# world-modelz/world-modelz

Measured on AMD Instinct MI355X. Metric: denoise-step latent-frames/sec (forward, 32x16x16 latent clips), higher is better.
Workload: dtype bf16; 1 GPU; BASELINE.json configs[3] per GPU: VqVideoDiffusionModel.forward, B=8 clips/GPU of 32x16x16 latents, codebook 1024, dim 256, dim_head 128, heads 1, extents 3,3,3, depth 4, mlp 256; clips_per_gpu=8, codebook=1024, parallelism=clips sharded over 1 rank(s), no data-path collective

## Files before the change

include/wmz.h:

```cpp
#ifndef WMZ_H_
#define WMZ_H_

#include <stdint.h>

#ifdef __cplusplus
extern "C" {
#endif

#define WMZ_VERSION 115

enum { WMZ_F32 = 0, WMZ_BF16 = 1,
       WMZ_F16 = 2  };
enum { WMZ_OK = 0, WMZ_ERR_ARG = 1, WMZ_ERR_HIP = 2, WMZ_ERR_UNSUPPORTED = 3 };

enum {
  WMZ_LIN_GELU = 1,
  WMZ_LIN_GELU_IN = 2,
  WMZ_LIN_DGELU = 4
};

int wmz_version(void);
const char* wmz_last_error(void);

enum { WMZ_HG_STREAM = 1 , WMZ_HG_QKV = 2 ,
       WMZ_HG_CONV = 4  };
int wmz_half_guard_bind(void* word);
int wmz_half_guard_clear(void* word, void* stream);

int wmz_local3d_attn_fwd(const void* q, const void* k, const void* v, void* out, float* lse, float* logits_dbg,
                         int B, int S, int H, int W, int heads, int dh, int eS, int eH, int eW,
                         long ldq, long ldk, long ldv, long ldo, int dtype, void* stream);

int wmz_local3d_attn_fwd_general(const void* q, const void* k, const void* v, void* out, float* lse, float* logits_dbg,
                                 int B, int S, int H, int W, int heads, int dh, int eS, int eH, int eW,
                                 long ldq, long ldk, long ldv, long ldo, int dtype, void* stream);

int wmz_local3d_attn_bwd(const void* q, const void* k, const void* v, const void* out, const float* lse,
                         const void* dout, void* dq, void* dk, void* dv, float* delta_ws,
                         int B, int S, int H, int W, int heads, int dh, int eS, int eH, int eW,
                         long ldq, long ldk, long ldv, long ldo, long lddo, long lddq, long lddk, long lddv,
                         int dtype, void* stream);

int wmz_local3d_attn_bwd_general(const void* q, const void* k, const void* v, const void* out, const float* lse,
                                 const void* dout, void* dq, void* dk, void* dv, float* delta_ws,
                                 int B, int S, int H, int W, int heads, int dh, int eS, int eH, int eW,
                                 long ldq, long ldk, long ldv, long ldo, long lddo, long lddq, long lddk, long lddv,
                                 int dtype, void* stream);

int wmz_linear_fwd(const void* A, long lda, const void* Wt, const float* bias, const void* residual, long ldr,
                   void* C, long ldc, int M, int N, int K, const float* ln_gamma, const float* ln_beta,
                   float ln_eps, int flags, int out_f32, int dtype, void* stream);

int wmz_linear_fwd_stats(const void* A, long lda, const void* Wt, const float* bias, const void* residual, long ldr,
                         void* C, long ldc, int M, int N, int K, const float* ln_gamma, const float* ln_beta,
                         const float* ln_mean, const float* ln_rstd, float ln_eps, int flags, int out_f32, int dtype,
                         void* stream);

int wmz_linear_fwd_gelu_pair(const void* A, long lda, const void* Wt, const float* bias, void* Z, long ldz, void* H, long ldh,
                             int M, int N, int K, const float* ln_gamma, const float* ln_beta, const float* ln_mean,
                             const float* ln_rstd, float ln_eps, int dtype, void* stream);
int wmz_linear_fwd_train(const void* A, long lda, const void* Wt, const float* bias, void* C, long ldc, void* H, long ldh,
                         void* An, long ldan, int M, int N, int K, const float* ln_gamma, const float* ln_beta,
                         const float* ln_mean, const float* ln_rstd, float ln_eps, int dtype, void* stream);

int wmz_linear_fwd_blocked(const void* A, long lda, int rows_per_block, long block_stride, const void* Wt,
                           const float* bias, void* C, long ldc, int M, int N, int K, int out_f32, int dtype, void* stream);

long wmz_linear_wgrad_workspace_floats(int M, int N, int K, int dtype);
int wmz_linear_wgrad_ws(const void* dC, long ldc, const void* A, long lda, float* dW, float* dbias, int M, int N, int K,
                        const float* ln_gamma, const float* ln_beta, const float* ln_mean, const float* ln_rstd,
                        int gelu_in, int overwrite, float* workspace, long workspace_floats, int dtype, void* stream);
int wmz_linear_wgrad_batch(int n, const void* const* dC, const long* ldc, const void* const* A, const long* lda,
                           float* const* dW, float* const* dbias, const int* M, const int* N, const int* K,
                           const int* overwrite, const int* a_tiled, float* workspace, long workspace_floats, int dtype,
                           void* stream);
int wmz_linear_wgrad_batch_ln(int n, const void* const* dC, const long* ldc, const void* const* A, const long* lda,
                              float* const* dW, float* const* dbias, const int* M, const int* N, const int* K,
                              const int* overwrite, const float* const* ln_gamma, const float* const* ln_beta,
                              const float* const* ln_mean, const float* const* ln_rstd, float* workspace, long workspace_floats,
                              int dtype, void* stream);
int wmz_layernorm_stats(const void* x, long ldx, float* mean, float* rstd, int M, int K, float eps, int dtype,
                        void* stream);
int wmz_layernorm_bwd(const void* x, long ldx, const void* dyhat, long lddy, const void* skip, long ldskip,
                      const void* skip2, long ldskip2, const float* gamma, void* dx, long lddx, float* dgamma,
                      float* dbeta, int M, int K, float eps, int dtype, void* stream);

int wmz_embed_pos3d_fwd(const int64_t* z, const float* emb, const float* pos_s, const float* pos_h,
                        const float* pos_w, void* x, int B, int S, int H, int W, int D, int num_classes,
                        int dtype, void* stream);
int wmz_embed_pos3d_bwd(const int64_t* z, const void* dx, float* demb, float* dpos_s, float* dpos_h, float* dpos_w,
                        int B, int S, int H, int W, int D, int num_classes, int dtype, void* stream);
long wmz_embed_pos3d_bwd_workspace_ints(int B, int S, int H, int W, int num_classes);
int wmz_embed_pos3d_bwd_sorted(const int64_t* z, const void* dx, float* demb, float* dpos_s, float* dpos_h, float* dpos_w,
                               int B, int S, int H, int W, int D, int num_classes, int* workspace, long workspace_ints,
                               int dtype, void* stream);

int wmz_embed_indexed_fwd(const int64_t* tok, const int64_t* pos, const float* emb, const float* pos_s,
                          const float* pos_h, const float* pos_w, void* x, long ntok, int S, int H, int W, int D,
                          int num_classes, int dtype, void* stream);
int wmz_embed_indexed_bwd(const int64_t* tok, const int64_t* pos, const void* dx, float* demb, float* dpos_s,
                          float* dpos_h, float* dpos_w, long ntok, int S, int H, int W, int D, int num_classes, int dtype,
                          void* stream);

int wmz_vq_argmin(const float* x, long ldx, const float* codebook, int64_t* idx, float* dist_min,
                  int N, int C, int E, void* stream);

long wmz_vq_argmin_screened_workspace_bytes(int N, int C, int E);
int wmz_vq_argmin_screened(const float* x, long ldx, const float* codebook, int64_t* idx, float* dist_min, int N, int C, int E,
                           void* workspace, long workspace_bytes, void* stream);
int wmz_vq_gather(const int64_t* idx, const float* codebook, void* out, long ldo, int N, int C, int E,
                  int dtype, void* stream);
long wmz_loss_partials_workspace_floats(void);
int wmz_vq_tail_fwd(const float* x, const float* q, const float* counts, void* st, float* partial, float* loss,
                    float* perplexity, long N, int E, int Ep, int C, int out_dtype, void* stream);
int wmz_vq_tail_bwd(const void* d_st, const float* x, const float* q, const float* g_loss, void* d_x, long N, int E, int Ep,
                    int in_dtype, int st_dtype, void* stream);
int wmz_recon_loss_fwd(const void* y, const float* target, float* partial, float* loss, long B, long HW, int C, int Cp,
                       int kind, int dtype, void* stream);
int wmz_recon_loss_bwd(const void* y, const float* target, const float* g_loss, void* d_y, long B, long HW, int C, int Cp,
                       int kind, int dtype, void* stream);
int wmz_vq_ema_stats(const float* x, long ldx, const int64_t* idx, const float* codebook, float* counts,
                     float* dw, float* sqerr, int N, int C, int E, void* stream);
long wmz_vq_ema_stats_workspace_ints(int N, int C);
int wmz_vq_ema_stats_sorted(const float* x, long ldx, const int64_t* idx, const float* codebook, float* counts, float* dw,
                            float* sqerr, int N, int C, int E, int* workspace, long workspace_ints, void* stream);
int wmz_vq_ema_update(float* embedding, float* cluster_size, float* activation_count, const float* counts,
                      const float* dw, int C, int E, double decay, double eps, void* stream);

int wmz_layer_fused_fwd(const void* o, const void* x, void* x_out, void* q_out, void* kv_out, const void* wpack,
                        const float* vec, int ntok, int D, int I, int M, int has_head, int has_tail, float eps,
                        void* stream);

int wmz_embed_qkv_fused_fwd(const int64_t* z, const float* emb, const float* pos_s, const float* pos_h,
                            const float* pos_w, void* x_out, void* q_out, void* kv_out, const void* wpack,
                            const float* vec, int B, int S, int H, int W, int D, int I, int M, int num_classes, float eps,
                            void* stream);

#define WMZ_FUSED_X_IN_TILED 1
#define WMZ_FUSED_X_OUT_TILED 2
#define WMZ_FUSED_X1_NORMALISED 4
#define WMZ_FUSED_XRM_NORMALISED 8
int wmz_local3d_attn_fwd_planes(const void* q, const void* k, const void* v, void* out, float* lse, int B, int S, int H,
                                int W, int heads, int dh, int eS, int eH, int eW, long ldq, long ldk, long ldv, long ldo,
                                int q_plane0, int q_planes, int dtype, void* stream);
int wmz_layer_fused_fwd_planes(const void* o, const void* x, void* x_out, void* q_out, void* kv_out, const void* wpack,
                               const float* vec, int B, int planes_out, int planes_in, int HW, int D, int I, int M,
                               int has_head, int has_tail, int xflags, float eps, void* stream);
int wmz_layer_chain_supported(int D, int I, int M, int* mc);
int wmz_layer_chain_slab_pieces(void);
// ... 239 lines not shown
```

world_modelz_amd/csrc/linear_fwd.hip:

```cpp
#include "wmz_common.h"

namespace {

constexpr int BN = 128, ROWB = 128, CPR = 8, NT = 256;

struct LinParams {
  const void* A; long lda;
  const void* Wt;
  const float* bias;
  const void* res; long ldr;
  void* C; long ldc;
  void* C2; long ldc2;
  void* An; long ldan;
  int M, N, K;
  const float* gamma; const float* beta; float eps;
  const float* mean; const float* rstd;
  int flags, out_f32;
  int nbn;
  int rpb; long bstride;
  int dma;
};

typedef const __attribute__((address_space(1))) void* gptr_t;
typedef __attribute__((address_space(3))) void* lptr_t;

template <int N>
__device__ __forceinline__ void lgkm_wait_for3(s16x8& a, s16x8& b, s16x8& c) {
  asm volatile("s_waitcnt lgkmcnt(%3)" : "+v"(a), "+v"(b), "+v"(c) : "n"(N) : "memory");
}

template <typename T> __device__ __forceinline__ const T* a_row(const LinParams& P, int m) {
  const T* A = reinterpret_cast<const T*>(P.A);
  if (P.rpb == 0) return A + (long)m * P.lda;
  const int blk = m / P.rpb;
  return A + (long)blk * P.bstride + (long)(m - blk * P.rpb) * P.lda;
}

template <typename T, int PRO, int BM>
__global__ __launch_bounds__(NT, 2) void linear_kernel(LinParams P) {
  constexpr bool LN = PRO == 1;
  constexpr int NJ = BM == 128 ? 2 : 1;
  constexpr int AI = BM / 32;
  constexpr int EPC = 16 / (int)sizeof(T);
  constexpr int BK = CPR * EPC;
  constexpr int KSTEPS = BK / 16;
  constexpr bool DMA_FORM = PRO == 0 && BM == 64 && sizeof(T) == 2;
  constexpr int SLAB = (BM + BN) * ROWB;
  __shared__ __attribute__((aligned(1024))) char tiles[(DMA_FORM ? 3 : 1) * SLAB];
  char* As = tiles;
  char* Bs = tiles + BM * ROWB;
  __shared__ float mean_s[BM], rstd_s[BM];

  const int tid = threadIdx.x, lane = tid & 63, wave = tid >> 6;
  const int lid = xcd_remap(blockIdx.x, gridDim.x);
  const int bm = lid / P.nbn, bn = lid - bm * P.nbn;
  const int m0 = bm * BM, n0 = bn * BN;
  const T* A = reinterpret_cast<const T*>(P.A);
  const T* Wt = reinterpret_cast<const T*>(P.Wt);
  const int K = P.K;

  if constexpr (LN) {
   if (P.mean != nullptr) {
    for (int r = tid; r < BM; r += NT) {
      const int gm = m0 + r < P.M ? m0 + r : P.M - 1;
      mean_s[r] = P.mean[gm];
      rstd_s[r] = P.rstd[gm];
    }
   } else {
    const int sub = tid & 7;
    for (int r = tid >> 3; r < BM; r += NT / 8) {
      const int gm = m0 + r;
      float sum = 0.f;
      if (gm < P.M) {
        const T* row = a_row<T>(P, gm);
        for (int c = sub; c * EPC < K; c += 8) {
          float f[EPC];
          Elem<T>::unpack(*reinterpret_cast<const i32x4*>(row + c * EPC), f);
#pragma unroll
          for (int i = 0; i < EPC; ++i) sum += f[i];
        }
      }
      sum += __shfl_xor(sum, 1); sum += __shfl_xor(sum, 2); sum += __shfl_xor(sum, 4);
      const float mean = sum / (float)K;
// ... 238 lines not shown
        }
        __syncthreads();
#pragma unroll
        for (int it = 0; it < RR / 16; ++it) {
          const int idx = tid + it * NT;
          const int rl = idx >> 4, ch = idx & 15;
          const int row = m0 + round * RR + rl, col = n0 + ch * 8;
          if (row >= P.M || col >= P.N) continue;
          const f32x4 a = *reinterpret_cast<const f32x4*>(stage + rl * BN + ch * 8);
          const f32x4 b = *reinterpret_cast<const f32x4*>(stage + rl * BN + ch * 8 + 4);
          float f[8] = {a[0], a[1], a[2], a[3], b[0], b[1], b[2], b[3]};
          if (f32_staged) {
            float* dstf = reinterpret_cast<float*>(P.C) + (long)row * P.ldc + col;
            if (col + 8 <= P.N) {
              *reinterpret_cast<f32x4*>(dstf) = a;
              *reinterpret_cast<f32x4*>(dstf + 4) = b;
            } else {
              for (int e = 0; e < 8 && col + e < P.N; ++e) dstf[e] = f[e];
            }
            continue;
          }
          T* dst = reinterpret_cast<T*>(P.C) + (long)row * P.ldc + col;
          if (col + 8 <= P.N) {
            if (R) {
              float r8[8];
              Elem<T>::unpack(*reinterpret_cast<const i32x4*>(R + (long)row * P.ldr + col), r8);
#pragma unroll
              for (int e = 0; e < 8; ++e) {
                if (dgelu) f[e] *= wmz_dgelu(r8[e]);
                else f[e] += r8[e];
              }
            }
            *reinterpret_cast<i32x4*>(dst) = Elem<T>::pack(f);
            if (P.C2) {
#pragma unroll
              for (int e = 0; e < 8; ++e) f[e] = wmz_gelu(f[e]);
              *reinterpret_cast<i32x4*>(reinterpret_cast<T*>(P.C2) + (long)row * P.ldc2 + col) = Elem<T>::pack(f);
            }
          } else {
            for (int e = 0; e < 8 && col + e < P.N; ++e) {
              float v = f[e];
              if (R) {
                const float rv = Elem<T>::to_f32(R[(long)row * P.ldr + col + e]);
                if (dgelu) v *= wmz_dgelu(rv);
                else v += rv;
              }
              dst[e] = Elem<T>::from_f32(v);
              if (P.C2) reinterpret_cast<T*>(P.C2)[(long)row * P.ldc2 + col + e] = Elem<T>::from_f32(wmz_gelu(v));
            }
          }
        }
      }
      return;
    }
  }
#pragma unroll
  for (int i = 0; i < 2; ++i)
#pragma unroll
    for (int j = 0; j < NJ; ++j) {
      const int col = n0 + wc + 32 * j + l31;
      if (col >= P.N) continue;
      const float bv = P.bias ? P.bias[col] : 0.f;
#pragma unroll
      for (int reg = 0; reg < 16; ++reg) {
        const int row = m0 + wr + 32 * i + (reg & 3) + 8 * (reg >> 2) + 4 * hh;
        if (row >= P.M) continue;
        float v = acc[i][j][reg] + bv;
        if (gelu) v = wmz_gelu(v);
        if (R) {
          const float rv = Elem<T>::to_f32(R[(long)row * P.ldr + col]);
          if (dgelu) {
            v *= wmz_dgelu(rv);
          } else {
            v += rv;
          }
        }
        if (P.out_f32) reinterpret_cast<float*>(P.C)[(long)row * P.ldc + col] = v;
        else reinterpret_cast<T*>(P.C)[(long)row * P.ldc + col] = Elem<T>::from_f32(v);
        if (P.C2) reinterpret_cast<T*>(P.C2)[(long)row * P.ldc2 + col] = Elem<T>::from_f32(wmz_gelu(v));
      }
    }
}

}

extern "C" int WMZ_FN(wmz_linear_fwd)(const void* A, long lda, const void* Wt, const float* bias, const void* residual,
                              long ldr, void* C, long ldc, int M, int N, int K, const float* ln_gamma,
                              const float* ln_beta, float ln_eps, int flags, int out_f32, int dtype, void* stream) {
  return WMZ_FN(wmz_linear_fwd_stats)(A, lda, Wt, bias, residual, ldr, C, ldc, M, N, K, ln_gamma, ln_beta, nullptr, nullptr, ln_eps,
                              flags, out_f32, dtype, stream);
}

static int g_linear_dma = 1;
#ifndef WMZ_OP16_F16
extern "C" int wmz_debug_linear_knobs(int dma) { g_linear_dma = dma; return WMZ_OK; }
#endif

struct LinRoute { bool small; int bm; int dma; };
static LinRoute linear_route(const LinParams& P, bool op16, bool ln, bool gin, int dma_knob) {
  LinRoute r;
  r.small = (long)wmz_cdiv(P.M, 128) * wmz_cdiv(P.N, BN) < (P.out_f32 ? 192 : 320) && (op16 || (!ln && !gin));
  r.bm = r.small ? 64 : 128;
  const uintptr_t al = (uintptr_t)P.A | (uintptr_t)P.Wt | (uintptr_t)(P.lda * 2) | (uintptr_t)(P.bstride * 2);
  r.dma = (r.small && op16 && !ln && !gin && P.K % 64 == 0 && (al & 15) == 0 && dma_knob) ? 1 : 0;
  return r;
}

#ifndef WMZ_OP16_F16
extern "C" int wmz_debug_linear_route(const void* A, long lda, const void* Wt, long block_stride, int M, int N, int K, int prologue,
                                      int out_f32, int dtype) {
  WMZ_REQUIRE(M > 0 && N > 0 && K > 0 && prologue >= 0 && prologue <= 2, "wmz_debug_linear_route: bad shape or prologue");
  WMZ_REQUIRE(dtype == WMZ_F32 || dtype == WMZ_BF16 || dtype == WMZ_F16, "wmz_debug_linear_route: bad dtype %d", dtype);
  LinParams P = {};
  P.A = A; P.lda = lda; P.Wt = Wt; P.bstride = block_stride; P.M = M; P.N = N; P.K = K; P.out_f32 = out_f32;
  const LinRoute r = linear_route(P, dtype != WMZ_F32, prologue == 1, prologue == 2, dtype == WMZ_F16 ? 1 : g_linear_dma);
  return r.bm | (r.dma << 8);
}
#endif

static int linear_launch(LinParams P, const float* ln_gamma, int flags, int dtype, hipStream_t st) {
  const bool ln = ln_gamma != nullptr;
  const bool gin = (flags & WMZ_LIN_GELU_IN) != 0;
  WMZ_REQUIRE(!(ln && gin), "wmz_linear_fwd: LayerNorm and GELU prologues are exclusive");
  P.nbn = wmz_cdiv(P.N, BN);
  const LinRoute route = linear_route(P, dtype == kOp16Dtype, ln, gin, g_linear_dma);
  const bool small = route.small;
  const int bm = route.bm;
  P.dma = route.dma;
  dim3 grid((unsigned)(wmz_cdiv(P.M, bm) * P.nbn)), block(NT);
  if (dtype == kOp16Dtype) {
    if (small && ln) hipLaunchKernelGGL((linear_kernel<bf16_t, 1, 64>), grid, block, 0, st, P);
    else if (small && gin) hipLaunchKernelGGL((linear_kernel<bf16_t, 2, 64>), grid, block, 0, st, P);
    else if (small) hipLaunchKernelGGL((linear_kernel<bf16_t, 0, 64>), grid, block, 0, st, P);
    else if (ln) hipLaunchKernelGGL((linear_kernel<bf16_t, 1, 128>), grid, block, 0, st, P);
    else if (gin) hipLaunchKernelGGL((linear_kernel<bf16_t, 2, 128>), grid, block, 0, st, P);
    else hipLaunchKernelGGL((linear_kernel<bf16_t, 0, 128>), grid, block, 0, st, P);
  } else {
    if (small) hipLaunchKernelGGL((linear_kernel<float, 0, 64>), grid, block, 0, st, P);
    else if (ln) hipLaunchKernelGGL((linear_kernel<float, 1, 128>), grid, block, 0, st, P);
    else if (gin) hipLaunchKernelGGL((linear_kernel<float, 2, 128>), grid, block, 0, st, P);
    else hipLaunchKernelGGL((linear_kernel<float, 0, 128>), grid, block, 0, st, P);
  }
  WMZ_LAUNCH_CHECK("wmz_linear_fwd");
  return WMZ_OK;
}

extern "C" int WMZ_FN(wmz_linear_fwd_stats)(const void* A, long lda, const void* Wt, const float* bias, const void* residual,
                                    long ldr, void* C, long ldc, int M, int N, int K, const float* ln_gamma,
                                    const float* ln_beta, const float* ln_mean, const float* ln_rstd, float ln_eps,
                                    int flags, int out_f32, int dtype, void* stream) {
  WMZ_REQUIRE(A && Wt && C, "wmz_linear_fwd: null tensor");
  WMZ_REQUIRE((ln_mean == nullptr) == (ln_rstd == nullptr), "wmz_linear_fwd: ln_mean and ln_rstd go together");
  WMZ_REQUIRE(ln_mean == nullptr || ln_gamma != nullptr, "wmz_linear_fwd: statistics without a LayerNorm prologue");
  WMZ_REQUIRE(M > 0 && N > 0 && K > 0, "wmz_linear_fwd: bad shape M=%d N=%d K=%d", M, N, K);
  WMZ_REQUIRE(K % 8 == 0 && lda % 8 == 0, "wmz_linear_fwd: K and lda must be multiples of 8 (K=%d lda=%ld)", K, lda);
  WMZ_REQUIRE(dtype == WMZ_F32 || dtype == kOp16Dtype, "wmz_linear_fwd: bad dtype %d", dtype);
  WMZ_REQUIRE((ln_gamma == nullptr) == (ln_beta == nullptr), "wmz_linear_fwd: ln_gamma and ln_beta go together");
  LinParams P;
  P.A = A; P.lda = lda; P.Wt = Wt; P.bias = bias; P.res = residual; P.ldr = ldr; P.C = C; P.ldc = ldc;
  P.M = M; P.N = N; P.K = K; P.gamma = ln_gamma; P.beta = ln_beta; P.eps = ln_eps; P.flags = flags;
  P.mean = ln_mean; P.rstd = ln_rstd;
  P.out_f32 = out_f32;
  P.rpb = 0; P.bstride = 0;
  P.C2 = nullptr; P.ldc2 = 0;
  P.An = nullptr; P.ldan = 0;
  return linear_launch(P, ln_gamma, flags, dtype, (hipStream_t)stream);
}

#ifndef WMZ_OP16_F16
extern "C" int wmz_linear_fwd_gelu_pair(const void* A, long lda, const void* Wt, const float* bias, void* Z, long ldz, void* H,
                                        long ldh, int M, int N, int K, const float* ln_gamma, const float* ln_beta,
                                        const float* ln_mean, const float* ln_rstd, float ln_eps, int dtype, void* stream) {
  WMZ_REQUIRE(A && Wt && Z && H, "wmz_linear_fwd_gelu_pair: null tensor");
  WMZ_REQUIRE((ln_mean == nullptr) == (ln_rstd == nullptr), "wmz_linear_fwd_gelu_pair: ln_mean and ln_rstd go together");
  WMZ_REQUIRE(ln_mean == nullptr || ln_gamma != nullptr, "wmz_linear_fwd_gelu_pair: statistics without a LayerNorm prologue");
  WMZ_REQUIRE(M > 0 && N > 0 && K > 0, "wmz_linear_fwd_gelu_pair: bad shape M=%d N=%d K=%d", M, N, K);
  WMZ_REQUIRE(K % 8 == 0 && lda % 8 == 0, "wmz_linear_fwd_gelu_pair: K and lda must be multiples of 8 (K=%d lda=%ld)", K, lda);
  WMZ_REQUIRE(dtype == WMZ_F32 || dtype == kOp16Dtype, "wmz_linear_fwd_gelu_pair: bad dtype %d", dtype);
  WMZ_REQUIRE((ln_gamma == nullptr) == (ln_beta == nullptr), "wmz_linear_fwd_gelu_pair: ln_gamma and ln_beta go together");
  LinParams P;
  P.A = A; P.lda = lda; P.Wt = Wt; P.bias = bias; P.res = nullptr; P.ldr = 0; P.C = Z; P.ldc = ldz;
  P.M = M; P.N = N; P.K = K; P.gamma = ln_gamma; P.beta = ln_beta; P.eps = ln_eps; P.flags = 0;
  P.mean = ln_mean; P.rstd = ln_rstd;
  P.out_f32 = 0;
  P.rpb = 0; P.bstride = 0;
  P.C2 = H; P.ldc2 = ldh;
  P.An = nullptr; P.ldan = 0;
  return linear_launch(P, ln_gamma, 0, dtype, (hipStream_t)stream);
}

extern "C" int wmz_linear_fwd_train(const void* A, long lda, const void* Wt, const float* bias, void* C, long ldc, void* H, long ldh,
                                    void* An, long ldan, int M, int N, int K, const float* ln_gamma, const float* ln_beta,
                                    const float* ln_mean, const float* ln_rstd, float ln_eps, int dtype, void* stream) {
  WMZ_REQUIRE(A && Wt && C && ln_gamma && ln_beta, "wmz_linear_fwd_train: null tensor (a LayerNorm prologue is required)");
  WMZ_REQUIRE((ln_mean == nullptr) == (ln_rstd == nullptr), "wmz_linear_fwd_train: ln_mean and ln_rstd go together");
  WMZ_REQUIRE(M > 0 && N > 0 && K > 0, "wmz_linear_fwd_train: bad shape M=%d N=%d K=%d", M, N, K);
  WMZ_REQUIRE(K % 8 == 0 && lda % 8 == 0 && (An == nullptr || ldan % 8 == 0), "wmz_linear_fwd_train: K, lda, ldan must be multiples of 8");
  WMZ_REQUIRE(dtype == WMZ_F32 || dtype == kOp16Dtype, "wmz_linear_fwd_train: bad dtype %d", dtype);
  LinParams P;
  P.A = A; P.lda = lda; P.Wt = Wt; P.bias = bias; P.res = nullptr; P.ldr = 0; P.C = C; P.ldc = ldc;
  P.M = M; P.N = N; P.K = K; P.gamma = ln_gamma; P.beta = ln_beta; P.eps = ln_eps; P.flags = 0;
  P.mean = ln_mean; P.rstd = ln_rstd;
  P.out_f32 = 0;
  P.rpb = 0; P.bstride = 0;
  P.C2 = H; P.ldc2 = ldh;
  P.An = An; P.ldan = ldan;
  return linear_launch(P, ln_gamma, 0, dtype, (hipStream_t)stream);
}

#endif

extern "C" int WMZ_FN(wmz_linear_fwd_blocked)(const void* A, long lda, int rows_per_block, long block_stride, const void* Wt,
                                      const float* bias, void* C, long ldc, int M, int N, int K, int out_f32, int dtype,
                                      void* stream) {
  WMZ_REQUIRE(A && Wt && C, "wmz_linear_fwd_blocked: null tensor");
  WMZ_REQUIRE(M > 0 && N > 0 && K > 0 && rows_per_block > 0, "wmz_linear_fwd_blocked: bad shape M=%d N=%d K=%d rows_per_block=%d", M, N, K, rows_per_block);
  WMZ_REQUIRE(K % 8 == 0 && lda % 8 == 0 && block_stride % 8 == 0, "wmz_linear_fwd_blocked: K, lda, block_stride must be multiples of 8");
  WMZ_REQUIRE(dtype == WMZ_F32 || dtype == kOp16Dtype, "wmz_linear_fwd_blocked: bad dtype %d", dtype);
  LinParams P;
  P.A = A; P.lda = lda; P.Wt = Wt; P.bias = bias; P.res = nullptr; P.ldr = 0; P.C = C; P.ldc = ldc;
  P.M = M; P.N = N; P.K = K; P.gamma = nullptr; P.beta = nullptr; P.eps = 0.f; P.flags = 0;
  P.mean = nullptr; P.rstd = nullptr;
  P.out_f32 = out_f32;
  P.rpb = rows_per_block; P.bstride = block_stride;
  P.C2 = nullptr; P.ldc2 = 0;
  P.An = nullptr; P.ldan = 0;
  return linear_launch(P, nullptr, 0, dtype, (hipStream_t)stream);
}
```

world_modelz_amd/csrc/wmz_debug.h:

```cpp
#pragma once
#ifdef __cplusplus
extern "C" {
#endif

int wmz_debug_fused_timestamps(void* buf);
int wmz_debug_fused_knobs(int dbg);
int wmz_debug_attn_timestamps(void* buf);
int wmz_debug_attn_knobs(int dbg, int variant);

int wmz_debug_conv_knobs(int skew, int dbg);

int wmz_debug_linear_knobs(int dma);
int wmz_debug_linear_route(const void* A, long lda, const void* Wt, long block_stride, int M, int N, int K, int prologue,
                           int out_f32, int dtype);

int wmz_debug_stamp(void* buf, int slot, void* stream);

int wmz_debug_conv_stamps(unsigned long long* out, int n);
int wmz_debug_w3_stamps(unsigned long long* out, int n);
int wmz_debug_attn_infer_stamps(unsigned long long* out, int n);

#ifdef __cplusplus
}
#endif
```

world_modelz_amd/functional.py:

```python
import torch

from . import _cast, ops
from .config import get_compute_dtype

LN_EPS = 1e-5


class _AttentionBlock(torch.autograd.Function):
    @staticmethod
    def forward(ctx, x_kv, x_q, ln_g, ln_b, wq, wk, wv, bv, wout, bout, residual, extents, heads, grad_on, same_src,
                res_is_xkv, out_f32=False):
        dt = x_kv.dtype
        I = wq.shape[0]
        ln = None if ln_g is None else (ln_g.detach(), ln_b.detach())
        wq_c = _cast.operand(wq, dt)
        wkv_c = _cast.operand((wk, wv), dt, 'kv', lambda a, b: torch.cat([a, b], dim=0))
        bkv = _cast.operand((bv,), torch.float32, 'bkv', lambda b: torch.cat([torch.zeros_like(b), b]))
        lead = x_q.shape[:-1]
        need_bwd = grad_on and any(ctx.needs_input_grad)
        stats = ops.layernorm_stats(x_kv, LN_EPS) if (need_bwd and ln is not None) else None
        q = ops.linear_fwd(x_q, wq_c)
        xn = None
        if stats is not None and x_kv.numel() // x_kv.shape[-1] >= ops.KEEP_NORM_MIN_ROWS:
            kv, _, xn = ops.linear_fwd_train(x_kv, wkv_c, bkv, ln, LN_EPS, stats, want_norm=True)
        else:
            kv = ops.linear_fwd(x_kv, wkv_c, bias=bkv, ln=ln, ln_eps=LN_EPS, ln_stats=stats)
        o, lse, _ = ops.local3d_attention_fwd(q, kv[..., :I], kv[..., I:], extents, heads, need_lse=need_bwd)
        if wout is not None:
            y = ops.linear_fwd(o, _cast.operand(wout, dt), bias=bout.detach(), residual=residual, out_f32=bool(out_f32) and not need_bwd)
        else:
            y = o if residual is None else o + residual
        if need_bwd:
            ctx.save_for_backward(x_kv, x_q, ln_g, ln_b, wq, wk, wv, bv, wout, bout, q, kv, o, lse)
            ctx.extents, ctx.heads, ctx.has_res = extents, heads, residual is not None
            ctx.ln_stats = stats
            ctx.xn = xn
            ctx.same_src, ctx.res_is_xkv = bool(same_src), bool(res_is_xkv)
        return y.reshape(*lead, y.shape[-1])

    @staticmethod
    def backward(ctx, dy):
        from . import backward as B
        return B.attention_block_backward(ctx, dy) + (None,)


class _FeedForwardBlock(torch.autograd.Function):
    @staticmethod
    def forward(ctx, x, ln_g, ln_b, w1, b1, w2, b2, residual, grad_on, res_is_x):
        dt = x.dtype
        ln = None if ln_g is None else (ln_g.detach(), ln_b.detach())
        need_bwd = grad_on and any(ctx.needs_input_grad)
        w1_c, w2_c = _cast.operand(w1, dt), _cast.operand(w2, dt)
        if need_bwd:
            stats = ops.layernorm_stats(x, LN_EPS) if ln is not None else None
            xn = None
            if ln is not None and x.numel() // x.shape[-1] >= ops.KEEP_NORM_MIN_ROWS:
                z, h, xn = ops.linear_fwd_train(x, w1_c, b1.detach(), ln, LN_EPS, stats, want_gelu=True, want_norm=True)
            else:
                z, h = ops.linear_fwd_gelu_pair(x, w1_c, bias=b1.detach(), ln=ln, ln_eps=LN_EPS, ln_stats=stats)
            y = ops.linear_fwd(h, w2_c, bias=b2.detach(), residual=residual)
            ctx.save_for_backward(x, ln_g, ln_b, w1, b1, w2, b2, z, h, xn)
            ctx.ln_stats = stats
            ctx.has_res = residual is not None
            ctx.res_is_x = bool(res_is_x)
        else:
            h = ops.linear_fwd(x, w1_c, bias=b1.detach(), ln=ln, ln_eps=LN_EPS, gelu=True)
            y = ops.linear_fwd(h, w2_c, bias=b2.detach(), residual=residual)
        return y

    @staticmethod
    def backward(ctx, dy):
        from . import backward as B
        return B.feed_forward_block_backward(ctx, dy)


class _Embed(torch.autograd.Function):
    @staticmethod
    def forward(ctx, z, emb, pos_s, pos_h, pos_w, dtype):
        x = ops.embed_pos3d_fwd(z, emb.detach(), pos_s.detach(), pos_h.detach(), pos_w.detach(), dtype)
        ctx.save_for_backward(z)
        ctx.params = (emb, pos_s, pos_h, pos_w)
        return x

    @staticmethod
    def backward(ctx, dx):
        from . import backward as B
        return B.embed_backward(ctx, dx)


class _Linear(torch.autograd.Function):

    @staticmethod
    def forward(ctx, x, w, b, out_f32):
        bias = None if b is None else b.detach()
        if x.dim() >= 3 and not x.is_contiguous() and x[0].is_contiguous() and x.stride(0) % 8 == 0:
            xb = x.view(x.shape[0], -1, x.shape[-1])
            y = ops.linear_fwd_blocks(xb, _cast.operand(w, x.dtype), bias, out_f32).view(*x.shape[:-1], w.shape[0])
        else:
            y = ops.linear_fwd(x, _cast.operand(w, x.dtype), bias=bias, out_f32=out_f32)
        ctx.save_for_backward(x, w, b)
        return y

    @staticmethod
    def backward(ctx, dy):
        from . import backward as B
        return B.linear_backward(ctx, dy)


def _as_compute(x):
    dt = get_compute_dtype()
    if not x.is_cuda:
        raise ops.L.WmzError('world_modelz_amd modules run on the GPU only (no CPU fallback); got a CPU tensor')
    return x if x.dtype == dt else x.to(dt)


def attention_block(x_kv, x_q, ln, wq, wk, wv, bv, wout, bout, residual, extents, heads, out_f32=False):
    g, b = (None, None) if ln is None else ln
    return _AttentionBlock.apply(x_kv, x_q, g, b, wq, wk, wv, bv, wout, bout, residual, tuple(int(e) for e in extents),
                                 int(heads), torch.is_grad_enabled(), x_q is x_kv, residual is x_kv, bool(out_f32))


def feed_forward_block(x, ln, w1, b1, w2, b2, residual):
    g, b = (None, None) if ln is None else ln
    return _FeedForwardBlock.apply(x, g, b, w1, b1, w2, b2, residual, torch.is_grad_enabled(), residual is x)


def embed_tokens(z, emb, pos_s, pos_h, pos_w):
    return _Embed.apply(z, emb, pos_s, pos_h, pos_w, get_compute_dtype())


def linear(x, w, b=None, out_f32=False):
    return _Linear.apply(x, w, b, out_f32)



def _dense_grid(n):
    if n % 16 == 0:
        return (1, n // 16, 16), (0, n // 16, 16)
    return (1, 1, n), (0, 0, n)


class _DenseAttentionBlock(torch.autograd.Function):

    @staticmethod
    def forward(ctx, x, ln_g, ln_b, wqkv, wout, bout, residual, heads, grad_on, res_is_x):
        dt = x.dtype
        B, n, _ = x.shape
        I = wqkv.shape[0] // 3
        ln = None if ln_g is None else (ln_g.detach(), ln_b.detach())
        need_bwd = grad_on and any(ctx.needs_input_grad)
        stats = ops.layernorm_stats(x, LN_EPS) if (ln is not None and need_bwd) else None
        qkv = ops.linear_fwd(x, _cast.operand(wqkv, dt), ln=ln, ln_eps=LN_EPS, ln_stats=stats)
        (S, H, W), ext = _dense_grid(n)
        g = qkv.view(B, S, H, W, 3 * I)
        o, lse, _ = ops.local3d_attention_fwd(g[..., :I], g[..., I:2 * I], g[..., 2 * I:], ext, heads, need_lse=need_bwd)
        o = o.view(B, n, I)
        if wout is not None:
            y = ops.linear_fwd(o, _cast.operand(wout, dt), bias=bout.detach(), residual=residual)
        else:
            y = o if residual is None else o + residual
        if need_bwd:
            ctx.save_for_backward(x, ln_g, ln_b, wqkv, wout, bout, qkv, o, lse)
            ctx.ln_stats = stats
            ctx.heads, ctx.has_res = heads, residual is not None
            ctx.res_is_x = bool(res_is_x)
        return y

    @staticmethod
    def backward(ctx, dy):
        from . import backward as Bk
        return Bk.dense_attention_block_backward(ctx, dy)


class _EmbedIndexed(torch.autograd.Function):
    @staticmethod
    def forward(ctx, tok, pos, emb, pos_s, pos_h, pos_w, shape, dtype):
        x = ops.embed_indexed_fwd(tok, pos, emb.detach(), pos_s.detach(), pos_h.detach(), pos_w.detach(), shape, dtype)
        ctx.save_for_backward(tok, pos)
# ... 28 lines not shown
```

world_modelz_amd/ops.py:

```python
import contextlib
import ctypes
import os

import torch

from . import _lib as L


def _rows(t):
    if t.stride(-1) != 1:
        t = t.contiguous()
    C = t.shape[-1]
    flat = t.reshape(-1, C) if t.is_contiguous() else None
    if flat is None:
        if t.dim() >= 2 and all(t.stride(i) == t.stride(i + 1) * t.shape[i + 1] for i in range(t.dim() - 2)):
            return t, t.numel() // C, t.stride(-2)
        t = t.contiguous()
        flat = t.reshape(-1, C)
    return t, flat.shape[0], C


def _out_rows(out, M, dtype):
    t, Mo, ld = _rows(out)
    assert Mo == M and t.data_ptr() == out.data_ptr() and out.dtype == dtype
# ... 46 lines not shown
    if ln_stats is not None:
        mean, rstd = ln_stats
        assert ln is not None and mean.numel() == M and rstd.numel() == M
    L.call(L.half_form('wmz_linear_fwd_stats', a.dtype), L.ptr(a), lda, L.ptr(weight), L.ptr(bias), L.ptr(residual), ldr, L.ptr(out), ldc,
           M, N, K, L.ptr(g), L.ptr(b), L.ptr(mean), L.ptr(rstd), float(ln_eps),
           (L.WMZ_LIN_GELU if gelu else 0) | (L.WMZ_LIN_GELU_IN if gelu_in else 0), 1 if out_f32 else 0, dt,
           L.stream())
    return out


KEEP_NORM_MIN_ROWS = 16384


def linear_fwd_train(a, weight, bias, ln, ln_eps=1e-5, ln_stats=None, want_gelu=False, want_norm=False, out=None):
    K = a.shape[-1]
    N = weight.shape[0]
    dt = L.dtype_code(a.dtype)
    assert weight.dtype == a.dtype and weight.is_contiguous() and weight.shape[1] == K and ln is not None
    a, M, lda = _rows(a)
    lead = a.shape[:-1]
    ldc = ldh = N
    ldan = K
    if out is not None:
        c, h, an = out
        assert (h is not None) == want_gelu and (an is not None) == want_norm
        c, ldc = _out_rows(c, M, a.dtype)
        if h is not None:
            h, ldh = _out_rows(h, M, a.dtype)
        if an is not None:
            an, ldan = _out_rows(an, M, a.dtype)
    else:
        c = torch.empty(lead + (N,), dtype=a.dtype, device=a.device)
        h = torch.empty(lead + (N,), dtype=a.dtype, device=a.device) if want_gelu else None
        an = torch.empty(lead + (K,), dtype=a.dtype, device=a.device) if want_norm else None
    g, b = ln
    mean = rstd = None
    if ln_stats is not None:
        mean, rstd = ln_stats
        assert mean.numel() == M and rstd.numel() == M
    assert bias is None or bias.dtype == torch.float32
    L.call('wmz_linear_fwd_train', L.ptr(a), lda, L.ptr(weight), L.ptr(bias), L.ptr(c), ldc, L.ptr(h), ldh, L.ptr(an), ldan, M, N, K,
           L.ptr(g), L.ptr(b), L.ptr(mean), L.ptr(rstd), float(ln_eps), dt, L.stream())
    return c, h, an


def linear_fwd_gelu_pair(a, weight, bias=None, ln=None, ln_eps=1e-5, ln_stats=None, out=None):
    K = a.shape[-1]
    N = weight.shape[0]
    dt = L.dtype_code(a.dtype)
    assert weight.dtype == a.dtype and weight.is_contiguous() and weight.shape[1] == K
    a, M, lda = _rows(a)
    lead = a.shape[:-1]
    ldz = ldh = N
    if out is not None:
        z, ldz = _out_rows(out[0], M, a.dtype)
        h, ldh = _out_rows(out[1], M, a.dtype)
    else:
        z = torch.empty(lead + (N,), dtype=a.dtype, device=a.device)
        h = torch.empty(lead + (N,), dtype=a.dtype, device=a.device)
    g = b = mean = rstd = None
    if ln is not None:
        g, b = ln
        assert g.dtype == torch.float32 and b.dtype == torch.float32
    if ln_stats is not None:
        mean, rstd = ln_stats
        assert ln is not None and mean.numel() == M and rstd.numel() == M
    assert bias is None or bias.dtype == torch.float32
    L.call('wmz_linear_fwd_gelu_pair', L.ptr(a), lda, L.ptr(weight), L.ptr(bias), L.ptr(z), ldz, L.ptr(h), ldh, M, N, K,
           L.ptr(g), L.ptr(b), L.ptr(mean), L.ptr(rstd), float(ln_eps), dt, L.stream())
    return z, h


def linear_fwd_blocks(a, weight, bias=None, out_f32=False, out=None):
    Bk, R, K = a.shape
    N = weight.shape[0]
    assert a.stride(2) == 1 and weight.dtype == a.dtype and weight.is_contiguous() and weight.shape[1] == K
    ldc = N
    if out is None:
        out = torch.empty((Bk, R, N), dtype=torch.float32 if out_f32 else a.dtype, device=a.device)
    else:
        out, ldc = _out_rows(out, Bk * R, torch.float32 if out_f32 else a.dtype)
    L.call(L.half_form('wmz_linear_fwd_blocked', a.dtype), L.ptr(a), a.stride(1), R, a.stride(0), L.ptr(weight), L.ptr(bias), L.ptr(out), ldc,
           Bk * R, N, K, 1 if out_f32 else 0, L.dtype_code(a.dtype), L.stream())
    return out


def embed_pos3d_fwd(z, emb, pos_s, pos_h, pos_w, dtype):
    B, S, H, W = z.shape
    D = emb.shape[1]
    z = z.contiguous()
    x = torch.empty((B, S, H, W, D), dtype=dtype, device=z.device)
    L.call('wmz_embed_pos3d_fwd', L.ptr(z), L.ptr(emb), L.ptr(pos_s), L.ptr(pos_h), L.ptr(pos_w), L.ptr(x),
           B, S, H, W, D, emb.shape[0], L.dtype_code(dtype), L.stream())
    return x


_vq_screen_ws = {}


def vq_argmin(x, codebook, need_dist=False, exact_scan=False):
    assert x.dtype == torch.float32 and codebook.dtype == torch.float32
    x, N, ldx = _rows(x)
    codebook = codebook.contiguous()
    C, E = codebook.shape
    idx = torch.empty((N,), dtype=torch.int64, device=x.device)
    dmin = torch.empty((N,), dtype=torch.float32, device=x.device) if need_dist else None
    need = 0 if (exact_scan or N == 0 or ldx % 4 or x.data_ptr() % 16) else L.lib().wmz_vq_argmin_screened_workspace_bytes(N, C, E)
    if need > 0:
        ws = _vq_screen_ws.get(x.device)
        if ws is None or ws.numel() < need:
            ws = _vq_screen_ws[x.device] = torch.empty(need, dtype=torch.uint8, device=x.device)
        L.call('wmz_vq_argmin_screened', L.ptr(x), ldx, L.ptr(codebook), L.ptr(idx), L.ptr(dmin), N, C, E, L.ptr(ws), ws.numel(),
               L.stream())
    else:
        L.call('wmz_vq_argmin', L.ptr(x), ldx, L.ptr(codebook), L.ptr(idx), L.ptr(dmin), N, C, E, L.stream())
    return (idx, dmin) if need_dist else idx


def vq_gather(idx, codebook, dtype=torch.float32):
    codebook = codebook.contiguous()
    C, E = codebook.shape
    flat = idx.reshape(-1).contiguous()
    out = torch.empty((flat.shape[0], E), dtype=dtype, device=idx.device)
    L.call('wmz_vq_gather', L.ptr(flat), L.ptr(codebook), L.ptr(out), E, flat.shape[0], C, E, L.dtype_code(dtype),
           L.stream())
    return out.reshape(*idx.shape, E)


_loss_partials = {}


def _partials(device):
    w = _loss_partials.get(device)
    if w is None:
        w = _loss_partials[device] = torch.empty(int(L.lib().wmz_loss_partials_workspace_floats()), dtype=torch.float32, device=device)
    return w


class _VqTail(torch.autograd.Function):

    @staticmethod
    def forward(ctx, inp, flat, q, counts, out_dtype, Ep):
        N, E = flat.shape
        dev = flat.device
        st = torch.empty(inp.shape[:-1] + (Ep,), dtype=out_dtype, device=dev)
        loss = torch.empty((), dtype=torch.float32, device=dev)
        ppl = torch.empty((), dtype=torch.float32, device=dev)
        L.call('wmz_vq_tail_fwd', L.ptr(flat), L.ptr(q), L.ptr(counts), L.ptr(st), L.ptr(_partials(dev)), L.ptr(loss), L.ptr(ppl),
               N, E, Ep, counts.numel(), L.dtype_code(out_dtype), L.stream())
        ctx.save_for_backward(flat, q)
        ctx.meta = (inp.shape, inp.dtype, Ep, out_dtype)
        ctx.mark_non_differentiable(ppl)
        return st, loss, ppl

    @staticmethod
    def backward(ctx, d_st, d_loss, _d_ppl):
        flat, q = ctx.saved_tensors
        shape, in_dtype, Ep, out_dtype = ctx.meta
        N, E = flat.shape
        if d_st is not None:
            d_st = d_st.contiguous()
            assert d_st.dtype == out_dtype
        if d_loss is not None:
            d_loss = d_loss.reshape(1).float()
        dx = torch.empty(shape, dtype=in_dtype, device=flat.device)
        L.call('wmz_vq_tail_bwd', L.ptr(d_st), L.ptr(flat), L.ptr(q), L.ptr(d_loss), L.ptr(dx), N, E, Ep, L.dtype_code(in_dtype),
# ... 913 lines not shown
```

Baseline: 821,800 latent-frames/s.

## Add specialized single-pass logits GEMM kernel for K=256 bf16 fp32-output projection

Adds a dedicated kernel for the final codebook logits projection (K=256, bf16 inputs, fp32 output). It loads the whole K extent for a 64x128 tile into LDS in one pass using direct global-to-LDS loads, runs MFMA over four K slabs with fine-grained waits, then stages the results through LDS so fp32 stores are coalesced. The Python linear path sends eligible out_f32 calls to it and falls back to the generic blocked linear otherwise. This targets the generic kernel's tiling overhead and uncoalesced fp32 output writes on a large M x 1024 output, at the cost of a single-occupancy, large-LDS kernel.

```diff
diff --git a/include/wmz.h b/include/wmz.h
--- a/include/wmz.h
+++ b/include/wmz.h
@@ -65,6 +65,11 @@
 
 int wmz_linear_fwd_blocked(const void* A, long lda, int rows_per_block, long block_stride, const void* Wt,
                            const float* bias, void* C, long ldc, int M, int N, int K, int out_f32, int dtype, void* stream);
+
+int wmz_logits_fwd(const void* A, long lda, int rows_per_block, long block_stride, const void* Wt, const float* bias, float* C,
+                   long ldc, int M, int N, int K, int dtype, void* stream);
+int wmz_logits_unit_takes(const void* A, long lda, int rows_per_block, long block_stride, const void* Wt, const void* C, long ldc,
+                          int M, int N, int K, int dtype);
 
 long wmz_linear_wgrad_workspace_floats(int M, int N, int K, int dtype);
 int wmz_linear_wgrad_ws(const void* dC, long ldc, const void* A, long lda, float* dW, float* dbias, int M, int N, int K,
diff --git a/world_modelz_amd/csrc/linear_fwd.hip b/world_modelz_amd/csrc/linear_fwd.hip
--- a/world_modelz_amd/csrc/linear_fwd.hip
+++ b/world_modelz_amd/csrc/linear_fwd.hip
@@ -1,4 +1,5 @@
 #include "wmz_common.h"
+#include "mem_policy.h"
 
 namespace {
 
@@ -403,6 +404,113 @@
     }
 }
 
+#ifndef WMZ_OP16_F16
+struct LogitsParams {
+  const char* A; long lda_b;
+  int rpb; long bstride_b;
+  const char* Wt;
+  const float* bias;
+  float* C; long ldc;
+  int nbn;
+};
+constexpr int LU_BM = 64, LU_K = 256, LU_SLABS = LU_K / 64;
+constexpr int LU_SLAB = (LU_BM + BN) * ROWB;
+constexpr int LU_PITCH = 40;
+constexpr int LU_STAGE = LU_BM * LU_PITCH * 4;
+constexpr int LU_LDS = LU_SLABS * LU_SLAB + 4 * LU_STAGE;
+
+__global__ __launch_bounds__(NT, 1) void logits_unit_kernel(LogitsParams P) {
+  extern __shared__ __attribute__((aligned(1024))) char lu_lds[];
+  const int tid = threadIdx.x, lane = tid & 63;
+  const int wave = __builtin_amdgcn_readfirstlane(tid >> 6);
+  const int lid = xcd_remap(blockIdx.x, gridDim.x);
+  const int bm = lid / P.nbn, bn = lid - bm * P.nbn;
+  const int m0 = bm * LU_BM, n0 = bn * BN;
+  const int blk = m0 / P.rpb;
+  const char* a0 = P.A + (long)blk * P.bstride_b + (long)(m0 - blk * P.rpb) * P.lda_b;
+  const char* w0 = P.Wt + (long)n0 * (LU_K * 2);
+  const int l31 = lane & 31, hh = lane >> 5;
+  const float bv = P.bias ? P.bias[n0 + wave * 32 + l31] : 0.f;
+
+  {
+    const int lr = lane >> 3, lc = lane & 7;
+    const char* asrc[2];
+    const char* bsrc[4];
+#pragma unroll
+    for (int q = 0; q < 2; ++q) {
+      const int r = 8 * (wave + 4 * q) + lr;
+      asrc[q] = a0 + (long)r * P.lda_b + ((lc ^ (swz128(r) >> 4)) << 4);
+    }
+#pragma unroll
+    for (int q = 0; q < 4; ++q) {
+      const int r = 8 * (wave + 4 * q) + lr;
+      bsrc[q] = w0 + r * (LU_K * 2) + ((lc ^ (swz128(r) >> 4)) << 4);
+    }
+#pragma unroll
+    for (int s = 0; s < LU_SLABS; ++s) {
+      char* dst = lu_lds + s * LU_SLAB;
+#pragma unroll
+      for (int q = 0; q < 2; ++q)
+        __builtin_amdgcn_global_load_lds((gptr_t)(asrc[q] + s * ROWB), (lptr_t)(dst + (wave + 4 * q) * 1024), 16, 0, 0);
+#pragma unroll
+      for (int q = 0; q < 4; ++q)
+        __builtin_amdgcn_global_load_lds((gptr_t)(bsrc[q] + s * ROWB), (lptr_t)(dst + LU_BM * ROWB + (wave + 4 * q) * 1024), 16, 0, 0);
+    }
+  }
+
+  f32x16 acc[2] = {(f32x16)(0.f), (f32x16)(0.f)};
+  unsigned aA[4];
+  {
+    const unsigned base = lds_addr(lu_lds) + (unsigned)l31 * ROWB;
+    const int t = (hh * 16) ^ swz128(l31);
+#pragma unroll
+    for (int kk = 0; kk < 4; ++kk) aA[kk] = base + (unsigned)((kk * 32) ^ t);
+  }
+  const unsigned wrow = (unsigned)(LU_BM * ROWB + wave * 32 * ROWB);
+  static_for<LU_SLABS>([&](auto sc) {
+    constexpr int S = decltype(sc)::value;
+    constexpr int OFF = (S & 1) * LU_SLAB;
+    asm volatile("s_waitcnt vmcnt(%0)" ::"n"(6 * (LU_SLABS - 1 - S)) : "memory");
+    __builtin_amdgcn_s_barrier();
+    s16x8 fa[4], fb[4], fw[4];
+    static_for<4>([&](auto kc) {
+      constexpr int kk = decltype(kc)::value;
+      const unsigned a = aA[kk] + (unsigned)((S >> 1) * 2 * LU_SLAB);
+      fa[kk] = ds_read_b128_asm<OFF>(a);
+      fb[kk] = ds_read_b128_asm<OFF + 32 * ROWB>(a);
+      fw[kk] = ds_read_b128_asm<OFF>(a + wrow);
+    });
+    static_for<4>([&](auto kc) {
+      constexpr int kk = decltype(kc)::value;
+      lgkm_wait_for3<3 * (3 - kk)>(fa[kk], fb[kk], fw[kk]);
+      Frag8<bf16_t> x0, x1, w;
+      x0.v = fa[kk]; x1.v = fb[kk]; w.v = fw[kk];
+      mma32(acc[0], x0, w);
+      mma32(acc[1], x1, w);
+    });
+  });
+
+  float* stage = reinterpret_cast<float*>(lu_lds + LU_SLABS * LU_SLAB + wave * LU_STAGE);
+#pragma unroll
+  for (int i = 0; i < 2; ++i)
+#pragma unroll
+    for (int reg = 0; reg < 16; ++reg)
+      stage[(32 * i + (reg & 3) + 8 * (reg >> 2) + 4 * hh) * LU_PITCH + l31] = acc[i][reg] + bv;
+  __builtin_amdgcn_fence(__ATOMIC_RELEASE, "wavefront");
+  __builtin_amdgcn_wave_barrier();
+  __builtin_amdgcn_fence(__ATOMIC_ACQUIRE, "wavefront");
+  char* cbase = reinterpret_cast<char*>(P.C + (long)m0 * P.ldc + n0 + wave * 32);
+  const int sr = lane >> 3, sch = lane & 7;
+  const unsigned ldc_b = (unsigned)P.ldc * 4u;
+#pragma unroll
+  for (int it = 0; it < LU_BM / 8; ++it) {
+    const int row = 8 * it + sr;
+    const f32x4 v = *reinterpret_cast<const f32x4*>(stage + row * LU_PITCH + 4 * sch);
+    gstore_at<MemPolicy::Plain>(cbase, (unsigned)row * ldc_b + (unsigned)sch * 16u, 0, v);
+  }
+}
+#endif
+
 }
 
 extern "C" int WMZ_FN(wmz_linear_fwd)(const void* A, long lda, const void* Wt, const float* bias, const void* residual,
@@ -548,3 +656,37 @@
   P.An = nullptr; P.ldan = 0;
   return linear_launch(P, nullptr, 0, dtype, (hipStream_t)stream);
 }
+
+#ifndef WMZ_OP16_F16
+extern "C" int wmz_logits_unit_takes(const void* A, long lda, int rows_per_block, long block_stride, const void* Wt, const void* C,
+                                     long ldc, int M, int N, int K, int dtype) {
+  if (dtype != WMZ_BF16 || K != LU_K || M <= 0 || N <= 0) return 0;
+  if (rows_per_block <= 0 || rows_per_block % LU_BM != 0 || M % rows_per_block != 0 || N % BN != 0) return 0;
+  if (ldc < N || ldc > (1L << 22) || lda < K) return 0;
+  const uintptr_t al = (uintptr_t)A | (uintptr_t)Wt | (uintptr_t)(lda * 2) | (uintptr_t)(block_stride * 2) | (uintptr_t)C |
+                       (uintptr_t)(ldc * 4);
+  return (al & 15) == 0 ? 1 : 0;
+}
+
+static int g_logits_keep_linear = 0;
+extern "C" int wmz_debug_logits_knobs(int keep_linear) { g_logits_keep_linear = keep_linear; return WMZ_OK; }
+extern "C" int wmz_debug_logits_route(const void* A, long lda, int rows_per_block, long block_stride, const void* Wt, const void* C,
+                                      long ldc, int M, int N, int K, int dtype) {
+  return !g_logits_keep_linear && wmz_logits_unit_takes(A, lda, rows_per_block, block_stride, Wt, C, ldc, M, N, K, dtype);
+}
+
+extern "C" int wmz_logits_fwd(const void* A, long lda, int rows_per_block, long block_stride, const void* Wt, const float* bias,
+                              float* C, long ldc, int M, int N, int K, int dtype, void* stream) {
+  if (g_logits_keep_linear || !wmz_logits_unit_takes(A, lda, rows_per_block, block_stride, Wt, C, ldc, M, N, K, dtype))
+    return wmz_linear_fwd_blocked(A, lda, rows_per_block, block_stride, Wt, bias, C, ldc, M, N, K, 1, dtype, stream);
+  static std::atomic<uint64_t> attr_devs{0};
+  if (wmz_first_use_on_device(attr_devs))
+    (void)hipFuncSetAttribute(reinterpret_cast<const void*>(&logits_unit_kernel), hipFuncAttributeMaxDynamicSharedMemorySize, 160 * 1024);
+  LogitsParams P;
+  P.A = reinterpret_cast<const char*>(A); P.lda_b = lda * 2; P.rpb = rows_per_block; P.bstride_b = block_stride * 2;
+  P.Wt = reinterpret_cast<const char*>(Wt); P.bias = bias; P.C = C; P.ldc = ldc; P.nbn = N / BN;
+  hipLaunchKernelGGL(logits_unit_kernel, dim3((unsigned)((M / LU_BM) * P.nbn)), dim3(NT), LU_LDS, (hipStream_t)stream, P);
+  WMZ_LAUNCH_CHECK("wmz_logits_fwd");
+  return WMZ_OK;
+}
+#endif
diff --git a/world_modelz_amd/csrc/wmz_debug.h b/world_modelz_amd/csrc/wmz_debug.h
--- a/world_modelz_amd/csrc/wmz_debug.h
+++ b/world_modelz_amd/csrc/wmz_debug.h
@@ -13,6 +13,9 @@
 int wmz_debug_linear_knobs(int dma);
 int wmz_debug_linear_route(const void* A, long lda, const void* Wt, long block_stride, int M, int N, int K, int prologue,
                            int out_f32, int dtype);
+int wmz_debug_logits_knobs(int keep_linear);
+int wmz_debug_logits_route(const void* A, long lda, int rows_per_block, long block_stride, const void* Wt, const void* C, long ldc,
+                           int M, int N, int K, int dtype);
 
 int wmz_debug_stamp(void* buf, int slot, void* stream);
 
diff --git a/world_modelz_amd/functional.py b/world_modelz_amd/functional.py
--- a/world_modelz_amd/functional.py
+++ b/world_modelz_amd/functional.py
@@ -93,7 +93,11 @@
     @staticmethod
     def forward(ctx, x, w, b, out_f32):
         bias = None if b is None else b.detach()
-        if x.dim() >= 3 and not x.is_contiguous() and x[0].is_contiguous() and x.stride(0) % 8 == 0:
+        blocks = x.dim() >= 3 and not x.is_contiguous() and x[0].is_contiguous() and x.stride(0) % 8 == 0
+        xl = x.view(x.shape[0] if blocks else 1, -1, x.shape[-1]) if out_f32 and (blocks or x.is_contiguous()) else None
+        if xl is not None and ops.logits_unit_takes(xl, _cast.operand(w, x.dtype)):
+            y = ops.logits_fwd_blocks(xl, _cast.operand(w, x.dtype), bias).view(*x.shape[:-1], w.shape[0])
+        elif blocks:
             xb = x.view(x.shape[0], -1, x.shape[-1])
             y = ops.linear_fwd_blocks(xb, _cast.operand(w, x.dtype), bias, out_f32).view(*x.shape[:-1], w.shape[0])
         else:
diff --git a/world_modelz_amd/ops.py b/world_modelz_amd/ops.py
--- a/world_modelz_amd/ops.py
+++ b/world_modelz_amd/ops.py
@@ -152,6 +152,32 @@
         out, ldc = _out_rows(out, Bk * R, torch.float32 if out_f32 else a.dtype)
     L.call(L.half_form('wmz_linear_fwd_blocked', a.dtype), L.ptr(a), a.stride(1), R, a.stride(0), L.ptr(weight), L.ptr(bias), L.ptr(out), ldc,
            Bk * R, N, K, 1 if out_f32 else 0, L.dtype_code(a.dtype), L.stream())
+    return out
+
+
+def logits_unit_takes(a, weight, out=None):
+    Bk, R, K = a.shape
+    N = weight.shape[0]
+    if a.dtype != torch.bfloat16 or a.stride(2) != 1:
+        return False
+    ldc = N if out is None else _out_rows(out, Bk * R, torch.float32)[1]
+    return bool(L.lib().wmz_logits_unit_takes(
+        a.data_ptr(), a.stride(1), R, a.stride(0), weight.data_ptr(), 0 if out is None else out.data_ptr(), ldc, Bk * R, N, K,
+        L.WMZ_BF16))
+
+
+def logits_fwd_blocks(a, weight, bias=None, out=None):
+    Bk, R, K = a.shape
+    N = weight.shape[0]
+    assert a.dtype != torch.float16 and a.stride(2) == 1 and weight.dtype == a.dtype and weight.is_contiguous() and weight.shape[1] == K
+    assert bias is None or bias.dtype == torch.float32
+    ldc = N
+    if out is None:
+        out = torch.empty((Bk, R, N), dtype=torch.float32, device=a.device)
+    else:
+        out, ldc = _out_rows(out, Bk * R, torch.float32)
+    L.call('wmz_logits_fwd', L.ptr(a), a.stride(1), R, a.stride(0), L.ptr(weight), L.ptr(bias), L.ptr(out), ldc,
+           Bk * R, N, K, L.dtype_code(a.dtype), L.stream())
     return out
 
 
```

Result: no change. 828,800 latent-frames/s (median of 6 runs) (+0.9%).
